# google/sbsim

Hardware: AMD Instinct MI355X
Metric: zone-updates/sec (env-steps/sec x 9 zones) at batch=64k buildings per GPU (higher is better)
Workload: dtype f64

## Files before the change

sbsim_amd/csrc/sb_device.h:

```cpp
#ifndef SBSIM_AMD_SB_DEVICE_H_
#define SBSIM_AMD_SB_DEVICE_H_

#include <hip/hip_runtime.h>

#include <stdint.h>

#include "sbsim_amd.h"

namespace sb {

constexpr double kCAir = 1006.0;
constexpr double kCWater = 4180.0;
constexpr double kRhoWater = 1000.0;
constexpr double kGravity = 9.8;
constexpr int kNScalOut = 16;
constexpr int kNScal = 20;
constexpr int kChunk = 8;
constexpr int kPad = 8;
constexpr double kAgeNone = -1e300;
__host__ __device__ inline bool age_is_none(double age) { return age < -1e200; }
constexpr int kModeMask = 0xff, kValveBit = 0x100;

struct Dev {
  int B, H, W, Z, N, Np, ncls, pitch, NL;
// ... 36 lines not shown
  int stream_ms;
  int n_ring;
  double n_ring_f64;
  int lw[4], l0[2], rowbase[2], nch[2];
  int lag;
  int nslots;
  float pred_haste;
  float pred_slack;
  int two_skip;
  float skip_kappa;
  int pred_first;
  int lds_reg_bytes;
  int wg_per_cu;
  int r_seam, r_A, r_zscr, r_xchg, r_zoff, r_zmode;
  int r_cmap;
  const unsigned long long *cmapS;
  const unsigned long long *amapS;
  const unsigned long long *zmapS;
  const int *cell_state;
  double *ring;
  double *temp;
  double *zmean;
  double *zair;
  double *damper;
  double *qz;
  int *mode;
  double *scal;
  struct Bld *bld;
  double *gtabg;
  double *zsum;
  double *gsum;
  int *nsw;
  int *next_b;
  int sweep_wgs;
  int *redo_ctr;
  int *redo_list;
  double *redo_scratch;
  int redo_mode;
  int roll_exact;
  int dbg_redo_mod;
  int O, col_ahu, col_blr, col_aux;
  const int *col_zone;
  const double *obs_mean, *obs_sigma;
  int n_src, n_hist, hist_normalize;
  const int *src_dest, *hist_col, *hist_off;
  const double *hist_bins;
  const int *act_kind, *act_zone;
  const double *act_lo, *act_hi;
  const int *zone_act;
  int n_damper_actions;
  long long *dbg;
  int dbg_timeline;
  sb_params p;
};

struct StepArgs {
  const float *actions;
  float *obs, *reward, *info;
  sb_step_in in;
};

int launch_sweep_lds(const Dev &d, int workgroups, int waves_per_wg, size_t lds_bytes, hipStream_t stream);
int prepare_sweep_lds(size_t lds_bytes);
int launch_sweep_reg(const Dev &d, int cus, hipStream_t stream);
int prepare_sweep_reg(const Dev &d);
bool sweep_reg_supported(int NR, int P);
int sweep_reg_table_stride(int NR, int P);
int sweep_reg_lds_slots(int NR, int P);
int sweep_reg_waves_per_simd(int NR, int P);
int launch_sweep_roll(const Dev &d, hipStream_t stream);
int launch_sweep_two(const Dev &d, hipStream_t stream);
int prepare_sweep_two(const Dev &d);
bool sweep_two_supported(int NR);
int sweep_two_levels();
int sweep_two_lds_slots(int NR, int level);
int sweep_two_a_stride(int NR, int level);
int sweep_two_seam_doubles(int NR);
int sweep_two_set_table();
int launch_sweep_band(const Dev &d, hipStream_t stream);
int prepare_sweep_band(const Dev &d);
bool sweep_band_supported(int NR);
int sweep_band_lds_slots(int NR);
int sweep_band_max_waves();
int sweep_band_seam_doubles(int NR, int W);
int sweep_band_sync_doubles(int W);
int sweep_band_decision_lag(int NR, int W);
int sweep_band_set_table();
int launch_sweep_stream(const Dev &d, double *abuf, int waves, hipStream_t stream);
int prepare_sweep_stream(const Dev &d, int waves);
int sweep_stream_set_table();
int sweep_stream_zone_columns();
int launch_sweep_stream_ms(const Dev &d, double *abuf, double *ebuf, int waves, hipStream_t stream);
int prepare_sweep_stream_ms(const Dev &d, int waves);
int sweep_stream_ms_sweeps();
int sweep_stream_ms_seam_doubles(int NS, int W);
int sweep_stream_ms_xchg_doubles(int W);
int prepare_sweep_roll(const Dev &d);
bool sweep_roll_supported(int NR);
int sweep_roll_lds_slots(int NR);
int sweep_roll_a_stride(int NR);
int sweep_roll_seam_doubles(int NR, int T);
int sweep_roll_waves();
int sweep_roll_tail_mul_doubles(int NR, int T);

template <int CTRL, int ROW_MASK>
__device__ __forceinline__ double dpp_or_zero(double x) {
// ... 442 lines not shown
```

sbsim_amd/csrc/sbsim_hip.hip:

```cpp
#include <hip/hip_runtime.h>

#include <algorithm>
#include <cmath>
#include <cstdio>
#include <cstdlib>
#include <cstring>
#include <memory>
#include <string>
#include <vector>

#include "sb_host.h"

#ifndef SB_EXPERIMENTAL
namespace sb {
int launch_sweep_stream_ms(const Dev &, double *, double *, int, hipStream_t) { return (int)hipErrorNotSupported; }
int prepare_sweep_stream_ms(const Dev &, int) { return (int)hipErrorNotSupported; }
int sweep_stream_ms_sweeps() { return 1; }
int sweep_stream_ms_seam_doubles(int, int) { return 0; }
int sweep_stream_ms_xchg_doubles(int) { return 0; }
}
#endif

using namespace sb;

namespace {

bool env_flag(const char *name) {
  const char *e = getenv(name);
  return e && e[0] == '1';
}
int env_int(const char *name, int unset) {
  const char *e = getenv(name);
  return e ? atoi(e) : unset;
}
double env_double(const char *name, double unset) {
  const char *e = getenv(name);
  return e ? atof(e) : unset;
}

struct Knobs {
  bool force_stream = env_flag("SBSIM_FORCE_STREAM_PATH");
  bool force_lds = env_flag("SBSIM_FORCE_LDS_PATH");
  bool band_path = env_flag("SBSIM_BAND_PATH");
  bool no_two_row = env_flag("SBSIM_NO_TWO_ROW_PATH");
  bool no_band = env_flag("SBSIM_NO_BAND_PATH");
  bool no_two_64 = env_flag("SBSIM_NO_TWO_64");
  bool no_roll_64 = env_flag("SBSIM_NO_ROLL_64");
  bool no_roll_small = env_flag("SBSIM_NO_ROLL_SMALL");
  bool two_general = env_flag("SBSIM_TWO_GENERAL");
  int two_max_level = std::max(0, env_int("SBSIM_TWO_MAX_LEVEL", 1 << 30));
  bool two_no_skip = env_flag("SBSIM_TWO_NO_SKIP");
  int lds_pad = env_int("SBSIM_DEBUG_LDS_PAD", 0);
  float pred_haste = (float)env_double("SBSIM_DEBUG_PRED_HASTE", 1.0);
  float pred_slack = (float)env_double("SBSIM_DEBUG_PRED_SLACK", 1.0);
  int pred_first = getenv("SBSIM_DEBUG_PRED_FIRST") ? std::max(1, env_int("SBSIM_DEBUG_PRED_FIRST", 1)) : 0;
  float skip_kappa = (float)std::min(100.0, std::max(0.0, env_double("SBSIM_DEBUG_SKIP_KAPPA", 0.9)));
  bool roll_exact = env_int("SBSIM_ROLL_EXACT", 0) != 0;
  int force_redo = std::max(0, env_int("SBSIM_DEBUG_FORCE_REDO", 0));
  bool force_generic = env_flag("SBSIM_FORCE_GENERIC_SWEEP");
  bool phase_timing = getenv("SBSIM_PHASE_TIMING") != nullptr;
  bool debug_timeline = getenv("SBSIM_DEBUG_TIMELINE") != nullptr;
  bool stream_ms = kExperimental && env_flag("SBSIM_STREAM_MS");
  bool stream_roll = kExperimental && env_flag("SBSIM_STREAM_ROLL");
};

constexpr int kGuardHost = 16;

struct RegPlan {
  bool ok = false;
  std::string why;
  sb_sweep_kernel kernel = SB_KERNEL_LDS;
  int NR = 0, RS = 0, Ws = 0, r0 = 0, c0 = 0, n_ring = 0, T = 0, state_doubles = 0, ts = 32;
  std::vector<uint8_t> tcls, tcset;
  std::vector<double> csetab;
  std::vector<double> tmul;
  int lw[4] = {0, 0, 0, 0}, l0[2] = {0, 0}, rowbase[2] = {0, 0}, nch[2] = {0, 0};
  int lag = 0, nslots = 0, steps = 0;
  int r_seam = 0, r_A = 0, r_xchg = 0, lds_bytes = 0, wg_per_cu = 0, AS = 0;
  int r_cmap = 0, wave_doubles = 0, waves_per_wg = 1;
  int ZRS = 0;
  int stream_variant = kStreamPlain;
  std::vector<unsigned long long> cmapS, amapS, zmapS;
  std::vector<int> cell_state;
  int two_sym = 0, two_level = 0, tail_set_base = 0, tail_pad_set = 0;
  std::vector<int> zs_off;
};

constexpr int kRegSeamPad = 8, kLdsCap = 160 * 1024;
constexpr int kLdsGranule = 1280;
constexpr int kRegSlots[] = {32, 66, 96};

int seam_lag(int lw0) { return (lw0 + 8) / 8 + 1; }

struct Trim {
  int x0, x1, y0, y1, Hs, Ws;
  std::vector<int> zone_of;
  std::string why;
};

Trim trim_box(const sb_plan_desc *plan) {
  const int H = plan->H, W = plan->W, ncls = plan->n_classes;
  auto coef = [&](int c, int j) { return plan->class_coef[c * 8 + j]; };
  auto cls_at = [&](int x, int y) { return (int)plan->cell_class[x * W + y]; };
  Trim t{H, -1, W, -1, 0, 0, std::vector<int>((size_t)H * W, -1), ""};
// ... 793 lines not shown
      return fail(SB_ERR_INVALID, "sb_create: unknown action kind");
    if (kind == SB_ACT_VAV_SUPPLY_AIR_DAMPER_COMMAND) {
      const int z = params->act_zone[i];
      if (z < 0 || z >= plan->Z) return fail(SB_ERR_INVALID, "sb_create: VAV action for a zone the floor plan does not have");
      if (acts.zone_act[z] >= 0) return fail(SB_ERR_INVALID, "sb_create: two action columns drive the same VAV damper");
      acts.zone_act[z] = i;
      ++acts.n_damper_actions;
    } else if (seen[kind]++) {
      return fail(SB_ERR_INVALID, "sb_create: two action columns drive the same setpoint");
    }
  }
  if (obs->n_obs < 1) return fail(SB_ERR_INVALID, "sb_create: empty observation layout");
  if (!obs->mean || !obs->sigma || (plan->Z > 0 && !obs->col_zone))
    return fail(SB_ERR_INVALID, "sb_create: null observation-layout table");
  {
    const int n_fields = obs->n_src ? obs->n_src : obs->n_obs, n_ahu = params->ahu_has_weather ? 9 : 8;
    bool ok = obs->col_ahu >= 0 && obs->col_ahu + n_ahu <= n_fields && obs->col_boiler >= 0 &&
              obs->col_boiler + 3 <= n_fields && obs->col_aux >= 0 && obs->col_aux + SB_NUM_AUX <= obs->n_obs;
    for (int z = 0; z < plan->Z; ++z) ok = ok && obs->col_zone[z] >= 0 && obs->col_zone[z] + 3 <= n_fields;
    if (!ok) return fail(SB_ERR_INVALID, "sb_create: observation columns outside the observation row");
  }
  for (int z = 0; z < plan->Z; ++z)
    if (plan->zone_off[z + 1] == plan->zone_off[z]) return fail(SB_ERR_INVALID, "sb_create: a zone without cells");
  if (obs->n_src) {
    const int n_dev_fields = 3 * plan->Z + (params->ahu_has_weather ? 9 : 8) + 3;
    if (obs->n_src != n_dev_fields || !obs->src_dest || obs->n_hist < 0 ||
        (obs->n_hist > 0 && (!obs->hist_col || !obs->hist_off || !obs->hist_bins)))
      return fail(SB_ERR_INVALID, "sb_create: inconsistent histogram-reducer layout");
    for (int i = 0; i < obs->n_src; ++i)
      if (obs->src_dest[i] >= obs->n_obs || obs->src_dest[i] < -obs->n_hist)
        return fail(SB_ERR_INVALID, "sb_create: histogram-reducer destination out of range");
    for (int j = 0; j < obs->n_hist; ++j) {
      const int n = obs->hist_off[j + 1] - obs->hist_off[j];
      if (n < 1 || obs->hist_col[j] < 0 || obs->hist_col[j] + n > obs->n_obs)
        return fail(SB_ERR_INVALID, "sb_create: histogram columns out of range");
    }
  }
  return SB_OK;
}

int setup_reg(sb_handle *h, const sb_plan_desc *plan, const RegPlan &r, const Knobs &k) {
  Dev &d = h->d;
  for (int g = 0; g < d.N; ++g) h->h_state_index[g] = r.cell_state[g];
  d.pitch = d.W; d.NL = d.N; d.ts = r.ts;
  d.NR = r.NR; d.RS = r.RS; d.Ws = r.Ws; d.n_ring = r.n_ring; d.n_ring_f64 = (double)r.n_ring;
  d.T = r.T; d.state_doubles = r.state_doubles; d.AS = r.AS; d.ZRS = r.ZRS ? r.ZRS : (r.RS | 1);
  for (int w = 0; w < 2; ++w) { d.l0[w] = r.l0[w]; d.rowbase[w] = r.rowbase[w]; d.nch[w] = r.nch[w]; }
  for (int w = 0; w < 4; ++w) d.lw[w] = r.lw[w];
  d.lag = r.lag; d.nslots = r.nslots; d.nsteps = r.steps;
  d.lds_reg_bytes = r.lds_bytes; d.wg_per_cu = r.wg_per_cu;
  d.r_seam = r.r_seam; d.r_A = r.r_A; d.r_xchg = r.r_xchg;
  if (h->kernel == SB_KERNEL_ROLL) { d.r_cmap = r.r_cmap; d.lds_wave_doubles = r.wave_doubles; }
  d.pred_haste = k.pred_haste; d.pred_slack = k.pred_slack;
  if (h->kernel == SB_KERNEL_TWO_ROWS && !k.two_no_skip) {
    bool mono = true;
    for (int c = 0; c < plan->n_classes; ++c) {
      double sum = 0.0;
      for (int j = 0; j < 4; ++j) { mono = mono && plan->class_coef[c * 8 + j] >= 0.0; sum += plan->class_coef[c * 8 + j]; }
      mono = mono && sum <= 1.0;
    }
    d.two_skip = mono ? 1 : 0;
  }
  d.skip_kappa = k.skip_kappa;
  d.pred_first = h->kernel == SB_KERNEL_BAND ? 2 : 3;
  if (k.pred_first) d.pred_first = k.pred_first;
  SB_CHECK(upload(h->zone_cells_l, plan->zone_cells, (size_t)plan->zone_off[plan->Z]));
  SB_CHECK(upload(h->cmapS, r.cmapS.data(), r.cmapS.size()));
  SB_CHECK(upload(h->amapS, r.amapS.data(), r.amapS.size()));
  SB_CHECK(upload(h->zmapS, r.zmapS.data(), r.zmapS.size()));
  SB_CHECK(upload(h->cell_state, r.cell_state.data(), r.cell_state.size()));
  SB_CHECK(alloc_zero(h->ring, (size_t)d.B * std::max(r.n_ring, 1)));
  SB_CHECK(upload(h->tcls, r.tcls.data(), r.tcls.size()));
  SB_CHECK(upload(h->tcset, r.tcset.data(), r.tcset.size()));
  SB_CHECK(upload(h->csetab, r.csetab.data(), r.csetab.size()));
  SB_CHECK(upload(h->tmul, r.tmul.data(), r.tmul.size()));
  d.tmulS = h->tmul.p; d.tmul_doubles = (int)r.tmul.size();
  d.tcset = h->tcset.p; d.csetab = h->csetab.p; d.ncset = (int)r.csetab.size() / 4;
  d.csetab_doubles = (int)r.csetab.size();
  d.two_sym = r.two_sym; d.two_level = r.two_level; d.tail_set_base = r.tail_set_base;
  d.tail_pad_set = h->kernel == SB_KERNEL_TWO_ROWS ? r.tail_pad_set : (d.ncset - 1) * 32;
  if (!r.zs_off.empty()) {
    SB_CHECK(upload(h->zs_off, r.zs_off.data(), r.zs_off.size()));
    d.zs_off = h->zs_off.p;
  }
  SB_CHECK(alloc_zero(h->temp, (size_t)d.B * d.state_doubles));
  if (h->kernel == SB_KERNEL_STREAM) {
    SB_CHECK(alloc_zero(h->abuf, (size_t)h->info.workgroups * d.state_doubles));
    if (h->stream_variant != kStreamPlain) SB_CHECK(alloc_zero(h->ebuf, (size_t)h->info.workgroups * d.state_doubles));
  }
  if (h->kernel == SB_KERNEL_TWO_ROWS) {
    SB_CHECK(alloc_zero(h->abuf, (size_t)h->info.workgroups * (size_t)std::max(1, d.NR - sweep_two_lds_slots(d.NR, d.two_level)) * 128));
    d.two_abuf = h->abuf.p;
  }
  if (h->kernel == SB_KERNEL_ROLL) {
    SB_CHECK(alloc_zero(h->redo_ctr, 2));
    SB_CHECK(alloc_zero(h->redo_list, (size_t)d.B));
    SB_CHECK(alloc_zero(h->redo_scratch, (size_t)h->info.workgroups * h->info.waves_per_workgroup * d.state_doubles));
    d.redo_ctr = h->redo_ctr.p; d.redo_list = h->redo_list.p; d.redo_scratch = h->redo_scratch.p;
    d.roll_exact = k.roll_exact; d.dbg_redo_mod = k.force_redo;
  }
  d.tcls = h->tcls.p;
  d.cmapS = h->cmapS.p; d.amapS = h->amapS.p; d.zmapS = h->zmapS.p; d.cell_state = h->cell_state.p;
  d.ring = h->ring.p;
  return SB_OK;
}

int setup_lds(sb_handle *h, const sb_plan_desc *plan, const LdsPlan &q, const Knobs &k) {
  Dev &d = h->d;
  for (int g = 0; g < d.N; ++g) h->h_state_index[g] = kPad + g;
  d.pitch = q.pitch; d.NL = q.NL; d.S = q.S; d.S_magic = q.S_magic; d.nsteps = q.nsteps;
  d.nbands = q.nbands; d.fast = q.fast; d.ts = q.ts;
  if (k.force_generic) d.fast = 0;
  d.off_agtab = q.off_agtab; d.off_zscr = q.off_zscr; d.off_zmode = q.off_zmode;
  d.lds_wave_doubles = q.lds_wave_doubles;
// ... 200 lines not shown
```

sbsim_amd/csrc/step_roll.hip:

```cpp
#include "sweep_common.h"

namespace sb {
namespace {

using namespace sweep;

#ifndef SB_ONE_WAIT
#define SB_ONE_WAIT 1
#endif
constexpr int kWin = 63;
constexpr int kTS = 32;
constexpr int kSeamPad = 8;

constexpr int lds_slots(int NR) { return NR >= 72 ? 72 : ((NR / 2) % 2 ? NR : NR + 2); }
constexpr int a_stride(int NR) { return NR >= 72 ? 70 : ((NR / 2) % 2 ? NR : NR + 2); }
constexpr int kWaves = 4;
constexpr int tail_row(int NR) { return NR + 4; }

struct PairBuf {
  d2 ud0, lr0, ud1, lr1;
  d2 A;
  d2 sm;
};

// ... 30 lines not shown
  unsigned off;
  if constexpr (j % 4 == 0) asm("v_lshlrev_b32_sdwa %0, 5, %1 dst_sel:DWORD dst_unused:UNUSED_PAD src0_sel:DWORD src1_sel:BYTE_0" : "=v"(off) : "v"(h));
  else if constexpr (j % 4 == 1) asm("v_lshlrev_b32_sdwa %0, 5, %1 dst_sel:DWORD dst_unused:UNUSED_PAD src0_sel:DWORD src1_sel:BYTE_1" : "=v"(off) : "v"(h));
  else if constexpr (j % 4 == 2) asm("v_lshlrev_b32_sdwa %0, 5, %1 dst_sel:DWORD dst_unused:UNUSED_PAD src0_sel:DWORD src1_sel:BYTE_2" : "=v"(off) : "v"(h));
  else asm("v_lshlrev_b32_sdwa %0, 5, %1 dst_sel:DWORD dst_unused:UNUSED_PAD src0_sel:DWORD src1_sel:BYTE_3" : "=v"(off) : "v"(h));
  return (lds_d2)off;
}

template <int NR, int S, bool SEAM, int NAR>
__device__ __forceinline__ void load_first(PairBuf &p, Ctx<NR> &x, const double (&Areg)[NAR]) {
#ifdef SB_EXP_NOCOEF
  p.ud0 = p.lr0 = x.kc;
  const lds_d2 ct = nullptr;
#else
  const lds_d2 ct = step_set<NR, S>(x);
  p.ud0 = ct[0];
#endif
#if defined(SB_EXP_ONECOEF)
  p.lr0 = p.ud0;
#elif !defined(SB_EXP_NOCOEF)
  p.lr0 = ct[1];
#endif
  constexpr int q = (S + 1) % NR, NL = lds_slots(NR), AS = a_stride(NR);
  static_assert(q % 2 == 0 && AS % 2 == 0, "pairs start at odd steps");
  if constexpr (q < AS) p.A = *(const d2 *)(x.Arow + q);
  else if constexpr (q < NL) p.A = *(const d2 *)(x.Aext + (q - AS));
  else p.A = d2{Areg[q - NL], Areg[q + 1 - NL]};
  if constexpr (SEAM && S >= kWin) p.sm = *(const d2 *)(x.seam + S);
  else p.sm = d2{0.0, 0.0};
}
template <int NR, int S>
__device__ __forceinline__ void load_second(PairBuf &p, Ctx<NR> &x) {
#ifdef SB_EXP_NOCOEF
  p.ud1 = p.lr1 = x.kc;
#else
  const lds_d2 ct = step_set<NR, S>(x);
  p.ud1 = ct[0];
#ifdef SB_EXP_ONECOEF
  p.lr1 = p.ud1;
#else
  p.lr1 = ct[1];
#endif
#endif
}

__device__ __forceinline__ void track(Acc &acc, double d) {
#ifdef SB_EXP_NOTRACK
  return;
#endif
  asm("v_max_f32 %0, %0, %1" : "+v"(acc.fin) : "v"(acc.tr));
  asm("v_max_f32_dpp %0, %0, |%1| wave_shr:1 row_mask:0xf bank_mask:0xf bound_ctrl:1" : "+v"(acc.tr) : "v"(__double2hiint(d)));
}

template <int NR, int S, bool EXACT>
__device__ __forceinline__ void step(double (&e)[NR], double (&bk)[kWin], d2 ud, d2 lr, double A,
                                     double sm, Acc &acc) {
  constexpr int r = S % NR, rm = (S + NR - 1) % NR, rp = (S + 1) % NR;
  const double Dn = wave_shift1<0x130, true>(e[rp], sm);
  double t;
  asm("v_fma_f64 %0, %1, %2, %3" : "=&v"(t) : "v"(ud.y), "v"(Dn), "v"(A));
  t = fma(lr.y, e[rp], t);
  const double U = wave_shift1<0x13c, false>(e[rm], 0.0);
  t = fma(lr.x, e[rm], t);
  const double nv = fma(ud.x, U, t);
#ifndef SB_EXP_NOSR
  if constexpr (S > kWin) {
    double &sr = (S - kWin - 1) % 2 == 0 ? acc.sre : acc.sro;
    sr = wave_shift1<0x138, true>(sr, U);
  }
#endif
  if constexpr (S < kWin) {
    const double sel = lanes_upto<S>() ? nv : e[r];
    if constexpr (EXACT) acc.cur = fmax(acc.cur, fabs(sel - e[r]));
    else track(acc, sel - e[r]);
    e[r] = sel;
  } else if constexpr (S < NR) {
    if constexpr (EXACT) acc.cur = fmax(acc.cur, fabs(nv - e[r]));
    else track(acc, nv - e[r]);
    e[r] = nv;
  } else if constexpr (!EXACT) {
    constexpr int J = S - NR;
    track(acc, nv - e[r]);
#ifndef SB_EXP_NOCOPY
    bk[J] = e[r];
#endif
    e[r] = nv;
  } else {
    constexpr int J = S - NR;
    const double d = nv - e[r];
    bk[J] = e[r];
    e[r] = nv;
    const double sd = __hiloint2double((__double2hiint(d) & 0x7fffffff) | acc.sg, __double2loint(d));
    acc.cur = fmax(acc.cur, sd);
    acc.neg = fmin(acc.neg, sd);
    if constexpr (J + 1 < kWin)
      acc.sg = __builtin_amdgcn_update_dpp(acc.sg, acc.sg, 0x138, 0xf, 0xf, false);
    asm volatile("" : "+v"(acc.cur), "+v"(acc.neg));
  }
}

constexpr int kA0 = 8;
template <int NR, int NAR>
struct APass {
  const unsigned long long (&cw)[(NR + 7) / 8];
  unsigned tbase;
  double *Aw, *Ax;
  double (&Areg)[NAR];
  template <int J>
  __device__ __forceinline__ d2 fetch() const {
    static_assert(kTS * 8 == 256, "a class byte (class * 8) is the byte offset into ap[] and into g[]");
    const unsigned h = (J & 7) < 4 ? (unsigned)cw[J >> 3] : (unsigned)(cw[J >> 3] >> 32);
    unsigned ad;
    if constexpr ((J & 3) == 0) asm("v_add_u32_sdwa %0, %1, %2 dst_sel:DWORD dst_unused:UNUSED_PAD src0_sel:DWORD src1_sel:BYTE_0" : "=v"(ad) : "s"(tbase), "v"(h));
    else if constexpr ((J & 3) == 1) asm("v_add_u32_sdwa %0, %1, %2 dst_sel:DWORD dst_unused:UNUSED_PAD src0_sel:DWORD src1_sel:BYTE_1" : "=v"(ad) : "s"(tbase), "v"(h));
    else if constexpr ((J & 3) == 2) asm("v_add_u32_sdwa %0, %1, %2 dst_sel:DWORD dst_unused:UNUSED_PAD src0_sel:DWORD src1_sel:BYTE_2" : "=v"(ad) : "s"(tbase), "v"(h));
    else asm("v_add_u32_sdwa %0, %1, %2 dst_sel:DWORD dst_unused:UNUSED_PAD src0_sel:DWORD src1_sel:BYTE_3" : "=v"(ad) : "s"(tbase), "v"(h));
    const __attribute__((address_space(3))) double *tp = (const __attribute__((address_space(3))) double *)ad;
    return d2{tp[0], tp[kTS]};
  }
  template <int J>
  __device__ __forceinline__ void put(const d2 &pg, const double &ej) const {
    constexpr int q = (J + 1) % NR, NL = lds_slots(NR), AS = a_stride(NR);
    double av;
    asm("v_fma_f64 %0, %1, %2, %3" : "=v"(av) : "v"(pg.x), "v"(ej), "v"(pg.y));
    if constexpr (q < AS) Aw[q] = av;
    else if constexpr (q < NL) Ax[q - AS] = av;
    else Areg[q - NL] = av;
  }
};

#ifndef SB_DEPTH
#define SB_DEPTH 1
#endif
constexpr int kDepth = SB_DEPTH;
constexpr int kBufs = kDepth + 1;
constexpr int pair_buf(int S) { return ((S - 1) / 2) % kBufs; }

template <int NR, int S, int S1, bool WRAP, bool EXACT, bool APASS, int NAR>
__device__ __forceinline__ void roll_pairs(double (&e)[NR], double (&bk)[kWin], double (&Areg)[NAR],
                                           PairBuf (&pb)[kBufs], Ctx<NR> &x, Acc &acc, const APass<NR, NAR> &ap) {
  if constexpr (S < S1) {
    constexpr bool wrapped = WRAP && S + 2 * kDepth >= S1;
    constexpr int N = wrapped ? S + 2 * kDepth - NR : S + 2 * kDepth;
    PairBuf &cur = pb[pair_buf(S)], &nxt = pb[pair_buf(N)];
#if SB_ONE_WAIT
    asm volatile("" ::"v"(cur.ud0.x), "v"(cur.A.x), "v"(cur.sm.x), "v"(cur.ud1.x), "v"(cur.lr1.x));
    __builtin_amdgcn_sched_barrier(0);
#endif
    load_first<NR, N, !wrapped>(nxt, x, Areg);
    constexpr int j0 = kA0 + 3 * ((S - 1) / 2);
    static_assert(!APASS || (S % 2 == 1 && j0 >= S + 2 * kDepth + 2), "a slot's A is written before the pair that reads it ahead");
    d2 pa0 = d2{0.0, 0.0}, pa1 = d2{0.0, 0.0}, pa2 = d2{0.0, 0.0};
    if constexpr (APASS && j0 < NR) pa0 = ap.template fetch<j0 < NR ? j0 : 0>();
    if constexpr (APASS && j0 + 1 < NR) pa1 = ap.template fetch<j0 + 1 < NR ? j0 + 1 : 0>();
    if constexpr (APASS && j0 + 2 < NR) pa2 = ap.template fetch<j0 + 2 < NR ? j0 + 2 : 0>();
    __builtin_amdgcn_sched_barrier(0);
    step<NR, S, EXACT>(e, bk, cur.ud0, cur.lr0, cur.A.x, cur.sm.x, acc);
    __builtin_amdgcn_sched_barrier(0);
    load_second<NR, N + 1>(nxt, x);
    __builtin_amdgcn_sched_barrier(0);
    step<NR, S + 1, EXACT>(e, bk, cur.ud1, cur.lr1, cur.A.y, cur.sm.y, acc);
    __builtin_amdgcn_sched_barrier(0);
    if constexpr (APASS && j0 < NR) ap.template put<j0 < NR ? j0 : 0>(pa0, e[j0 < NR ? j0 : 0]);
    if constexpr (APASS && j0 + 1 < NR) ap.template put<j0 + 1 < NR ? j0 + 1 : 0>(pa1, e[j0 + 1 < NR ? j0 + 1 : 0]);
    if constexpr (APASS && j0 + 2 < NR) ap.template put<j0 + 2 < NR ? j0 + 2 : 0>(pa2, e[j0 + 2 < NR ? j0 + 2 : 0]);
    if constexpr (APASS) __builtin_amdgcn_sched_barrier(0);
    roll_pairs<NR, S + 2, S1, WRAP, EXACT, APASS>(e, bk, Areg, pb, x, acc, ap);
  }
}

template <int NR, int J>
__device__ __forceinline__ void hand_over(double (&e)[NR], const double (&bk)[kWin], const unsigned long long (&zw)[NR / 8],
                                          double *tp, const double *np_, double *zrow) {
  static_assert(NR % 8 == 0, "whole zone words");
  if constexpr (J < NR) {
    if constexpr (J < kWin) e[J] = lanes_upto<J>() ? bk[J] : e[J];
    if constexpr (J + 1 < kWin) e[J + 1] = lanes_upto<J + 1>() ? bk[J + 1] : e[J + 1];
    const unsigned w = (J & 7) < 4 ? (unsigned)zw[J / 8] : (unsigned)(zw[J / 8] >> 32);
    const unsigned off0 = (w >> (8 * (J & 3))) & 0xffu, off1 = (w >> (8 * ((J + 1) & 3))) & 0xffu;
#ifndef SB_EXP_NOMEM
    __builtin_nontemporal_store(d2{e[J], e[J + 1]}, (d2 *)(tp + J * 64));
#endif
    __hip_atomic_fetch_add((double *)((char *)zrow + off0), e[J], __ATOMIC_RELAXED, __HIP_MEMORY_SCOPE_WORKGROUP);
    __hip_atomic_fetch_add((double *)((char *)zrow + off1), e[J + 1], __ATOMIC_RELAXED, __HIP_MEMORY_SCOPE_WORKGROUP);
#ifndef SB_EXP_NOMEM
    const d2 nv = __builtin_nontemporal_load((const d2 *)(np_ + J * 64));
    e[J] = nv.x;
    e[J + 1] = nv.y;
#endif
    if constexpr ((J & 7) == 6) __builtin_amdgcn_sched_barrier(0);
    hand_over<NR, J + 2>(e, bk, zw, tp, np_, zrow);
  }
}

extern __shared__ __attribute__((aligned(16))) double lds[];

template <int NR, bool EXACT>
__global__ void __launch_bounds__(64 * kWaves) __attribute__((amdgpu_waves_per_eu(1, 1))) k_sweep_roll(Dev a) {
  const int nB = a.redo_mode ? __builtin_amdgcn_readfirstlane(a.redo_ctr[0]) : a.B;
  if (nB == 0) return;
  const int lane = threadIdx.x & 63;
  const int wave = __builtin_amdgcn_readfirstlane((int)threadIdx.x >> 6);
  const int gw = (int)blockIdx.x * kWaves + wave;
  constexpr int kASlots = (NR + 7) / 8, kZSlots = NR / 8, kCW = NR / 8;
  static_assert((NR / 2) % kBufs == 0, "pair buffers rotate through a whole period: pair_buf() must not alias across the wrap");
  constexpr int kNL = lds_slots(NR), kAS = a_stride(NR), kNAR = NR - kNL > 0 ? NR - kNL : 2;

  double *tabc = lds;
  unsigned long long *ctab8 = (unsigned long long *)(lds + a.r_cmap);
  double *tmul = lds + a.r_cmap + kCW * 64;
  double *wl = tmul + a.tmul_doubles + (size_t)wave * a.lds_wave_doubles;
  double *tapg = wl;
  double *tE0 = wl + a.r_seam + 2;
  double *A = wl + a.r_A;
  for (int i = threadIdx.x; i < a.lds_reg_bytes / 8; i += blockDim.x) lds[i] = 0.0;
  __syncthreads();
  for (int i = threadIdx.x; i < 4 * kTS; i += blockDim.x) tabc[i] = i < 4 * a.ncset ? a.csetab[i] : 0.0;
  for (int i = threadIdx.x; i < kCW * 64; i += blockDim.x) ctab8[i] = a.cmapS[i];
  for (int i = threadIdx.x; i < a.tmul_doubles; i += blockDim.x) tmul[i] = a.tmulS[i];
  if (lane < kTS) tapg[lane] = lane <= a.ncls ? a.ctab[lane * 8 + 4] : 0.0;
// ... 19 lines not shown
#pragma unroll
  for (int t = 0; t < kTailMax; ++t) {
    tset[t] = (a.ncset - 1) * 32 * 0x10001;
    tcls8[t] = (8 * a.ncls) | ((8 * a.ncls) << 8);
    if (t < a.T && tactive) {
      const int c0 = tc0, c1 = tc0 + 1;
      tset[t] = ((int)a.tcset[t * NR + c0] << 2) | ((int)a.tcset[t * NR + c1] << 18);
      tcls8[t] = (int)a.tcls[t * NR + c0] | ((int)a.tcls[t * NR + c1] << 8);
    }
  }
  const unsigned long long *amap = a.amapS + lane;
  const unsigned long long *zmap = a.zmapS + lane;

#ifdef SB_PHASE_STAMPS
#define SB_STAMP(i) do { if (a.dbg && gw == 0 && iter == 10 && lane == 0) a.dbg[i] = (long long)__builtin_readcyclecounter(); } while (0)
#else
#define SB_STAMP(i) do { } while (0)
#endif

  double e[NR];
  double nx_g = 0.0, nx_tail[kTailMax][2] = {{0.0, 0.0}, {0.0, 0.0}}, nx_tnow = 0.0, nx_lo = 0.0, nx_hi = 0.0;
#define SB_LOAD_AUX(bb)                                                                         \
  do {                                                                                          \
    nx_tnow = a.bld[(bb)].t_now;                                                                \
    nx_lo = a.scal[(size_t)(bb) * kNScal + 16];                                                 \
    nx_hi = a.scal[(size_t)(bb) * kNScal + 17];                                                 \
    nx_g = a.gtabg[(size_t)(bb) * kTS + (opaque(lane) & (kTS - 1))];  \
    const double *tt_ = a.temp + (size_t)(bb) * a.state_doubles + NR * 64;                      \
    _Pragma("unroll") for (int t = 0; t < kTailMax; ++t)                                        \
      _Pragma("unroll") for (int k = 0; k < 2; ++k)                                             \
        if (t < a.T) nx_tail[t][k] = tt_[t * NR + tc0 + k];                                     \
  } while (0)
  auto building = [&](int s) { return a.redo_mode ? __builtin_amdgcn_readfirstlane(a.redo_list[s]) : s; };
  const int b_first = gw < nB ? building(gw) : 0;
  if (gw < nB) {
    const double *tp_ = a.temp + (size_t)b_first * a.state_doubles;
#pragma unroll
    for (int j = 0; j < NR; j += 2) {
      const d2 v = __builtin_nontemporal_load((const d2 *)(tp_ + j * 64 + 2 * R));
      e[j] = v.x;
      e[j + 1] = v.y;
    }
    SB_LOAD_AUX(b_first);
  }
  unsigned long long amapw[kASlots];
#define SB_LOAD_AMAP(g0, g1)                                                                    \
  do {                                                                                          \
    const int o_ = opaque(0);                                                                   \
    _Pragma("unroll") for (int g = (g0); g < (g1); ++g) amapw[g] = amap[o_ + g * 64];           \
  } while (0)
  constexpr int kAHalf = kASlots / 2;
  SB_LOAD_AMAP(0, kASlots);
  int iter = 0;
  for (int s = gw, sn = 0, b = b_first, bn = 0; s < nB; s = sn, b = bn, ++iter) {
    int nb = 0;
    if (lane == 0) nb = atomicAdd(a.next_b, 1);
    SB_STAMP(0);
    x.wn = x.cw[0];
    __builtin_amdgcn_sched_barrier(0);
    const double t_now = nx_tnow;
    const double ring_d = a.n_ring > 0 ? fmax(fabs(t_now - nx_lo), fabs(t_now - nx_hi)) : 0.0;
    if (lane < kTS) tapg[kTS + opaque(lane)] = nx_g;
    double tv[kTailMax][2];
#pragma unroll
    for (int t = 0; t < kTailMax; ++t)
#pragma unroll
      for (int k = 0; k < 2; ++k) tv[t][k] = tactive ? nx_tail[t][k] : 0.0;
    *(d2 *)(tE0 + opaque(tcw)) = d2{tv[0][0], tv[0][1]};
    __builtin_amdgcn_wave_barrier();
    __builtin_amdgcn_sched_barrier(0);
    SB_STAMP(1);
    double At[kTailMax][2] = {{0.0, 0.0}, {0.0, 0.0}};
    if constexpr (!EXACT) {
      const double *pg[kTailMax][2];
#pragma unroll
      for (int t = 0; t < kTailMax; ++t)
#pragma unroll
        for (int k = 0; k < 2; ++k) pg[t][k] = (const double *)((const char *)tapg + ((opaque(tcls8[t]) >> (8 * k)) & 0xff));
      double tap[kTailMax][2], tg[kTailMax][2];
#pragma unroll
      for (int t = 0; t < kTailMax; ++t)
#pragma unroll
        for (int k = 0; k < 2; ++k) { tap[t][k] = pg[t][k][0]; tg[t][k] = pg[t][k][kTS]; }
#pragma unroll
      for (int t = 0; t < kTailMax; ++t)
#pragma unroll
        for (int k = 0; k < 2; ++k) At[t][k] = fma(tap[t][k], tv[t][k], tg[t][k]);
    } else {
#pragma unroll
      for (int t = 0; t < kTailMax; ++t)
#pragma unroll
        for (int k = 0; k < 2; ++k)
          if (t < a.T && tactive) {
            const int c8 = (opaque(tcls8[t]) >> (8 * k)) & 0xff;
            const double *pg = (const double *)((const char *)tapg + c8);
            At[t][k] = fma(pg[0], tv[t][k], pg[kTS]);
          }
    }

    double Areg[kNAR];
    Areg[0] = 0.0;
    const APass<NR, kNAR> ap{amapw, (unsigned)(size_t)(__attribute__((address_space(3))) double *)tapg, A + (size_t)R * kAS,
                             A + 64 * kAS + (size_t)R * (kNL - kAS), Areg};
    {
      static_assert(kA0 == 8 && kA0 + 3 * ((kWin - 1) / 2) >= NR, "the ramp-up's pairs reach the last slot");
      const d2 g0 = ap.template fetch<0>(), g1 = ap.template fetch<1>(), g2 = ap.template fetch<2>(), g3 = ap.template fetch<3>(),
               g4 = ap.template fetch<4>(), g5 = ap.template fetch<5>(), g6 = ap.template fetch<6>(), g7 = ap.template fetch<7>();
      __builtin_amdgcn_sched_barrier(0);
      ap.template put<0>(g0, e[0]); ap.template put<1>(g1, e[1]); ap.template put<2>(g2, e[2]); ap.template put<3>(g3, e[3]);
      ap.template put<4>(g4, e[4]); ap.template put<5>(g5, e[5]); ap.template put<6>(g6, e[6]); ap.template put<7>(g7, e[7]);
    }
    __builtin_amdgcn_wave_barrier();
    __builtin_amdgcn_sched_barrier(0);
    SB_STAMP(2);

    int n_sweeps = 0, converged = 0, redo = 0;
    double bk[kWin];
    {
      PairBuf pb[kBufs];
      Acc acc;
      acc.cur = 0.0; acc.neg = 0.0; acc.sg = lane == 0 ? (int)0x80000000 : 0;
      acc.tr = acc.fin = 0;
      acc.sre = acc.sro = 0.0;
      {
        const lds_d2 ct = step_set<NR, 0>(x);
        const d2 ud = ct[0], lr = ct[1];
        load_first<NR, 1, true>(pb[pair_buf(1)], x, Areg);
        load_second<NR, 2>(pb[pair_buf(1)], x);
        if constexpr (kDepth > 1) {
          load_first<NR, 3, true>(pb[pair_buf(3)], x, Areg);
          load_second<NR, 4>(pb[pair_buf(3)], x);
        }
        static_assert(kDepth <= 2, "initial fill of the pair buffers");
        step<NR, 0, EXACT>(e, bk, ud, lr, x.Arow[1], 0.0, acc);
      }
      __builtin_amdgcn_sched_barrier(0);
      roll_pairs<NR, 1, kWin, false, EXACT, true>(e, bk, Areg, pb, x, acc, ap);
#ifndef SB_STAMP_NEXT
      SB_STAMP(15);
#endif
#pragma nounroll
      for (;;) {
        __builtin_amdgcn_sched_barrier(0);
#ifdef SB_PHASE_STAMPS
#ifndef SB_STAMP_SWEEP
#define SB_STAMP_SWEEP 1
#endif
#define SB_STAMP2(i) do { if (a.dbg && gw == 0 && iter == 10 && sweep_idx == SB_STAMP_SWEEP && lane == 0) a.dbg[i] = (long long)__builtin_readcyclecounter(); } while (0)
        const int sweep_idx = n_sweeps;
#ifdef SB_STAMP_NEXT
        if (a.dbg && gw == 0 && iter == 10 && sweep_idx == SB_STAMP_SWEEP + 1 && lane == 0) a.dbg[15] = (long long)__builtin_readcyclecounter();
#endif
#else
#define SB_STAMP2(i) do { } while (0)
#endif
        SB_STAMP2(10);
        roll_pairs<NR, kWin, NR + kWin, true, EXACT, false>(e, bk, Areg, pb, x, acc, ap);
        SB_STAMP2(11);
        double U0, U1;
        {
          constexpr int last = (NR + kWin - 1) % NR;
          const double ul = wave_shift1<0x13c, false>(e[last], 0.0);
          double &sr = (NR - 1) % 2 == 0 ? acc.sre : acc.sro;
          sr = wave_shift1<0x138, true>(sr, ul);
          const int rev = (63 - lane) * 4;
          U0 = __hiloint2double(__builtin_amdgcn_ds_bpermute(rev, __double2hiint(acc.sre)),
                                __builtin_amdgcn_ds_bpermute(rev, __double2loint(acc.sre)));
          U1 = __hiloint2double(__builtin_amdgcn_ds_bpermute(rev, __double2hiint(acc.sro)),
                                __builtin_amdgcn_ds_bpermute(rev, __double2loint(acc.sro)));
        }
        SB_STAMP2(12);
        const double dt_ = tail_pass_static<NR>(a.T, tmul + opaque(tc0), tE0 + opaque(tcw), U0, U1, tv, tset, At);

        SB_STAMP2(13);
        if constexpr (EXACT) {
          double md = wave_max(fmax(acc.cur, dt_));
          if (n_sweeps == 0) md = fmax(md, ring_d);
          ++n_sweeps;
          converged = md <= p.conv_threshold;
        } else {
          asm("v_max_f32 %0, %0, %1" : "+v"(acc.fin) : "v"(acc.tr));
          int m_hi = max(__builtin_amdgcn_readlane(acc.fin, 63), wave_max_i32(__double2hiint(dt_)));
          if (n_sweeps == 0) m_hi = max(m_hi, __double2hiint(ring_d));
          const int thr_hi = __double2hiint(p.conv_threshold);
          ++n_sweeps;
          acc.fin = 0;
          acc.tr = lanes_upto<62>() ? acc.tr : 0;
          const bool undecided = m_hi == thr_hi || (a.dbg_redo_mod > 0 && b % a.dbg_redo_mod == 0);
          if (m_hi <= thr_hi && undecided) { redo = 1; break; }
          converged = m_hi < thr_hi;
        }
        SB_STAMP2(14);
#ifdef SB_EXP_DESYNC
        if (n_sweeps >= 1 + (int)(((unsigned)b * 2654435761u >> 13) % 9u)) break;
#else
        if (converged || n_sweeps >= p.iter_limit) break;
#endif
        pb[pair_buf(kWin)].sm = *(const d2 *)(x.seam + kWin);
        if constexpr (kDepth > 1) pb[pair_buf(kWin + 2)].sm = *(const d2 *)(x.seam + kWin + 2);
        acc.cur = -acc.neg;
        acc.neg = 0.0;
        acc.sg = lane == 0 ? (int)0x80000000 : 0;
      }
    }
    __builtin_amdgcn_sched_barrier(0);
    SB_STAMP(3);
    sn = a.sweep_wgs + __builtin_amdgcn_readfirstlane(nb);
    bn = sn < nB ? building(sn) : 0;
    if (sn < nB) SB_LOAD_AUX(bn);
    SB_LOAD_AMAP(0, kAHalf);
    __builtin_amdgcn_sched_barrier(0);
    SB_STAMP(4);

    double *zs = A;
    const int ZRS = a.ZRS;
    {
      unsigned long long zw[kZSlots];
      const unsigned long long *zm = zmap + opaque(0);
#pragma unroll
      for (int g = 0; g < kZSlots; ++g) zw[g] = zm[g * 64];
      __builtin_amdgcn_sched_barrier(0);
      double *tp = redo ? a.redo_scratch + (size_t)gw * a.state_doubles : a.temp + (size_t)b * a.state_doubles;
      double *Ttail = tp + NR * 64;
      double *zrow = zs + (size_t)opaque(R) * ZRS;
      for (int z = 0; z <= a.Z; ++z) zrow[z] = 0.0;
      __builtin_amdgcn_wave_barrier();
#pragma unroll
      for (int t = 0; t < kTailMax; ++t)
        if (t < a.T && tactive) {
          *(d2 *)(Ttail + t * NR + tc0) = d2{tv[t][0], tv[t][1]};
          zrow[a.Z] += tv[t][0] + tv[t][1];
        }
      const double *np_ = a.temp + (size_t)(sn < nB ? bn : b) * a.state_doubles;
      static_assert(RS == 64, "hand_over: slot stride");
      hand_over<NR, 0>(e, bk, zw, tp + 2 * R, np_ + 2 * R, zrow);
    }
    __builtin_amdgcn_sched_barrier(0);
    SB_STAMP(5);
    SB_LOAD_AMAP(kAHalf, kASlots);
    __builtin_amdgcn_sched_barrier(0);
    SB_STAMP(6);
    __builtin_amdgcn_wave_barrier();
    SB_STAMP(7);

    {
      double gacc = 0.0;
      for (int zb = 0; zb <= a.Z; zb += 16) {
        const int zz = zb + (lane >> 2), g = lane & 3;
        const double *zr = zs + (size_t)g * ZRS + (zz <= a.Z ? zz : a.Z);
        double part[RS / 4];
#pragma unroll
        for (int k = 0; k < RS / 4; ++k) part[k] = zr[(size_t)4 * k * ZRS];
        double v = 0.0;
#pragma unroll
        for (int k = 0; k < RS / 4; ++k) v += part[k];
        if (zz > a.Z) v = 0.0;
        v += dpp_or_zero<0xB1, 0xf>(v);
        v += dpp_or_zero<0x4E, 0xf>(v);
        if (g == 0 && zz < a.Z && !redo) a.zsum[(size_t)b * a.Z + zz] = v;
        if (g == 0 && zz <= a.Z) gacc += v;
      }
      const double gsum = wave_sum(gacc);
      if (lane == 0 && !redo) {
        a.gsum[b] = gsum + a.n_ring_f64 * t_now;
        a.nsw[b] = n_sweeps | (converged << 16);
      }
      if (lane == 0 && redo) a.redo_list[atomicAdd(a.redo_ctr, 1)] = b;
      SB_STAMP(8);
#ifdef SB_PHASE_STAMPS
      if (a.dbg && gw == 0 && iter == 10 && lane == 0) a.dbg[9] = n_sweeps;
#endif
    }
  }
#undef SB_STAMP
#undef SB_LOAD_AUX
#undef SB_LOAD_AMAP
}

}

bool sweep_roll_supported(int NR) { return NR == 64 || NR == 72 || NR == 80 || NR == 88 || NR == 96; }
int sweep_roll_lds_slots(int NR) { return lds_slots(NR); }
int sweep_roll_a_stride(int NR) { return a_stride(NR); }
int sweep_roll_seam_doubles(int NR, int T) { (void)T; return tail_row(NR); }
int sweep_roll_waves() { return kWaves; }
int sweep_roll_tail_mul_doubles(int NR, int T) { return tail_mul_doubles(NR, T); }

int sweep_roll_redo_workgroups() { return 8; }

namespace {

template <int NR>
int prepare(const Dev &d) {
  const int e = (int)hipFuncSetAttribute((const void *)k_sweep_roll<NR, false>, hipFuncAttributeMaxDynamicSharedMemorySize,
                                         d.lds_reg_bytes);
  if (e != (int)hipSuccess) return e;
  return (int)hipFuncSetAttribute((const void *)k_sweep_roll<NR, true>, hipFuncAttributeMaxDynamicSharedMemorySize,
                                  d.lds_reg_bytes);
}

template <int NR>
int launch(const Dev &d, hipStream_t stream) {
  const dim3 grid((d.sweep_wgs + kWaves - 1) / kWaves), block(64 * kWaves);
  if (d.roll_exact) {
    hipLaunchKernelGGL((k_sweep_roll<NR, true>), grid, block, (size_t)d.lds_reg_bytes, stream, d);
    return (int)hipGetLastError();
  }
  hipLaunchKernelGGL((k_sweep_roll<NR, false>), grid, block, (size_t)d.lds_reg_bytes, stream, d);
  Dev r = d;
  r.redo_mode = 1;
  r.next_b = d.redo_ctr + 1;
  r.sweep_wgs = sweep_roll_redo_workgroups() * kWaves;
  hipLaunchKernelGGL((k_sweep_roll<NR, true>), dim3(sweep_roll_redo_workgroups()), block, (size_t)d.lds_reg_bytes, stream, r);
  return (int)hipGetLastError();
}

// ... 22 lines not shown
```

Measured before the change: 285.8 million.

## Skip convergence measurement on predicted non-converging sweeps in roll kernel

Extends the measurement-skip scheme from the two-row kernel to the roll kernel. The code extrapolates the residual decay from the last two measured sweeps, predicts how many sweeps remain, and runs those sweeps without residual tracking or backup copies. If a skipped run overshoots convergence, the building is rerun from scratch with full measurement, holding its slot instead of drawing new work. This removes per-sweep tracking and backup cost, at the price of more control flow and occasional full reruns.

```diff
diff --git a/sbsim_amd/csrc/sb_device.h b/sbsim_amd/csrc/sb_device.h
--- a/sbsim_amd/csrc/sb_device.h
+++ b/sbsim_amd/csrc/sb_device.h
@@ -112,6 +112,7 @@
   long long *dbg;
   int dbg_timeline;
   sb_params p;
+  int roll_skip;
 };
 
 struct StepArgs {
diff --git a/sbsim_amd/csrc/sbsim_hip.hip b/sbsim_amd/csrc/sbsim_hip.hip
--- a/sbsim_amd/csrc/sbsim_hip.hip
+++ b/sbsim_amd/csrc/sbsim_hip.hip
@@ -50,6 +50,7 @@
   bool two_general = env_flag("SBSIM_TWO_GENERAL");
   int two_max_level = std::max(0, env_int("SBSIM_TWO_MAX_LEVEL", 1 << 30));
   bool two_no_skip = env_flag("SBSIM_TWO_NO_SKIP");
+  bool roll_no_skip = env_flag("SBSIM_ROLL_NO_SKIP");
   int lds_pad = env_int("SBSIM_DEBUG_LDS_PAD", 0);
   float pred_haste = (float)env_double("SBSIM_DEBUG_PRED_HASTE", 1.0);
   float pred_slack = (float)env_double("SBSIM_DEBUG_PRED_SLACK", 1.0);
@@ -949,14 +950,14 @@
   d.r_seam = r.r_seam; d.r_A = r.r_A; d.r_xchg = r.r_xchg;
   if (h->kernel == SB_KERNEL_ROLL) { d.r_cmap = r.r_cmap; d.lds_wave_doubles = r.wave_doubles; }
   d.pred_haste = k.pred_haste; d.pred_slack = k.pred_slack;
-  if (h->kernel == SB_KERNEL_TWO_ROWS && !k.two_no_skip) {
+  if ((h->kernel == SB_KERNEL_TWO_ROWS && !k.two_no_skip) || (h->kernel == SB_KERNEL_ROLL && !k.roll_no_skip)) {
     bool mono = true;
     for (int c = 0; c < plan->n_classes; ++c) {
       double sum = 0.0;
       for (int j = 0; j < 4; ++j) { mono = mono && plan->class_coef[c * 8 + j] >= 0.0; sum += plan->class_coef[c * 8 + j]; }
       mono = mono && sum <= 1.0;
     }
-    d.two_skip = mono ? 1 : 0;
+    (h->kernel == SB_KERNEL_ROLL ? d.roll_skip : d.two_skip) = mono ? 1 : 0;
   }
   d.skip_kappa = k.skip_kappa;
   d.pred_first = h->kernel == SB_KERNEL_BAND ? 2 : 3;
diff --git a/sbsim_amd/csrc/step_roll.hip b/sbsim_amd/csrc/step_roll.hip
--- a/sbsim_amd/csrc/step_roll.hip
+++ b/sbsim_amd/csrc/step_roll.hip
@@ -106,9 +106,10 @@
   asm("v_max_f32_dpp %0, %0, |%1| wave_shr:1 row_mask:0xf bank_mask:0xf bound_ctrl:1" : "+v"(acc.tr) : "v"(__double2hiint(d)));
 }
 
-template <int NR, int S, bool EXACT>
+template <int NR, int S, bool EXACT, bool MEAS = true>
 __device__ __forceinline__ void step(double (&e)[NR], double (&bk)[kWin], d2 ud, d2 lr, double A,
                                      double sm, Acc &acc) {
+  static_assert(MEAS || (!EXACT && S >= kWin), "only the library kernel's rolling periods run measure-free");
   constexpr int r = S % NR, rm = (S + NR - 1) % NR, rp = (S + 1) % NR;
   const double Dn = wave_shift1<0x130, true>(e[rp], sm);
   double t;
@@ -130,14 +131,17 @@
     e[r] = sel;
   } else if constexpr (S < NR) {
     if constexpr (EXACT) acc.cur = fmax(acc.cur, fabs(nv - e[r]));
-    else track(acc, nv - e[r]);
+    else if constexpr (MEAS) track(acc, nv - e[r]);
     e[r] = nv;
   } else if constexpr (!EXACT) {
     constexpr int J = S - NR;
-    track(acc, nv - e[r]);
+    if constexpr (MEAS) {
+      track(acc, nv - e[r]);
 #ifndef SB_EXP_NOCOPY
-    bk[J] = e[r];
-#endif
+      bk[J] = e[r];
+#endif
+    }
+    (void)J;
     e[r] = nv;
   } else {
     constexpr int J = S - NR;
@@ -190,7 +194,7 @@
 constexpr int kBufs = kDepth + 1;
 constexpr int pair_buf(int S) { return ((S - 1) / 2) % kBufs; }
 
-template <int NR, int S, int S1, bool WRAP, bool EXACT, bool APASS, int NAR>
+template <int NR, int S, int S1, bool WRAP, bool EXACT, bool APASS, bool MEAS = true, int NAR>
 __device__ __forceinline__ void roll_pairs(double (&e)[NR], double (&bk)[kWin], double (&Areg)[NAR],
                                            PairBuf (&pb)[kBufs], Ctx<NR> &x, Acc &acc, const APass<NR, NAR> &ap) {
   if constexpr (S < S1) {
@@ -209,17 +213,17 @@
     if constexpr (APASS && j0 + 1 < NR) pa1 = ap.template fetch<j0 + 1 < NR ? j0 + 1 : 0>();
     if constexpr (APASS && j0 + 2 < NR) pa2 = ap.template fetch<j0 + 2 < NR ? j0 + 2 : 0>();
     __builtin_amdgcn_sched_barrier(0);
-    step<NR, S, EXACT>(e, bk, cur.ud0, cur.lr0, cur.A.x, cur.sm.x, acc);
+    step<NR, S, EXACT, MEAS>(e, bk, cur.ud0, cur.lr0, cur.A.x, cur.sm.x, acc);
     __builtin_amdgcn_sched_barrier(0);
     load_second<NR, N + 1>(nxt, x);
     __builtin_amdgcn_sched_barrier(0);
-    step<NR, S + 1, EXACT>(e, bk, cur.ud1, cur.lr1, cur.A.y, cur.sm.y, acc);
+    step<NR, S + 1, EXACT, MEAS>(e, bk, cur.ud1, cur.lr1, cur.A.y, cur.sm.y, acc);
     __builtin_amdgcn_sched_barrier(0);
     if constexpr (APASS && j0 < NR) ap.template put<j0 < NR ? j0 : 0>(pa0, e[j0 < NR ? j0 : 0]);
     if constexpr (APASS && j0 + 1 < NR) ap.template put<j0 + 1 < NR ? j0 + 1 : 0>(pa1, e[j0 + 1 < NR ? j0 + 1 : 0]);
     if constexpr (APASS && j0 + 2 < NR) ap.template put<j0 + 2 < NR ? j0 + 2 : 0>(pa2, e[j0 + 2 < NR ? j0 + 2 : 0]);
     if constexpr (APASS) __builtin_amdgcn_sched_barrier(0);
-    roll_pairs<NR, S + 2, S1, WRAP, EXACT, APASS>(e, bk, Areg, pb, x, acc, ap);
+    roll_pairs<NR, S + 2, S1, WRAP, EXACT, APASS, MEAS>(e, bk, Areg, pb, x, acc, ap);
   }
 }
 
@@ -345,9 +349,11 @@
   constexpr int kAHalf = kASlots / 2;
   SB_LOAD_AMAP(0, kASlots);
   int iter = 0;
+  int held = -1;
   for (int s = gw, sn = 0, b = b_first, bn = 0; s < nB; s = sn, b = bn, ++iter) {
     int nb = 0;
-    if (lane == 0) nb = atomicAdd(a.next_b, 1);
+    if (lane == 0 && (EXACT || held < 0)) nb = atomicAdd(a.next_b, 1);
+    const bool all_meas = held >= 0;
     SB_STAMP(0);
     x.wn = x.cw[0];
     __builtin_amdgcn_sched_barrier(0);
@@ -407,7 +413,7 @@
     __builtin_amdgcn_sched_barrier(0);
     SB_STAMP(2);
 
-    int n_sweeps = 0, converged = 0, redo = 0;
+    int n_sweeps = 0, converged = 0, redo = 0, rerun = 0;
     double bk[kWin];
     {
       PairBuf pb[kBufs];
@@ -432,21 +438,62 @@
 #ifndef SB_STAMP_NEXT
       SB_STAMP(15);
 #endif
+#ifdef SB_PHASE_STAMPS
+#ifndef SB_STAMP_SWEEP
+#define SB_STAMP_SWEEP 1
+#endif
+#define SB_STAMP2(i) do { if (a.dbg && gw == 0 && iter == 10 && sweep_idx == SB_STAMP_SWEEP && lane == 0) a.dbg[i] = (long long)__builtin_readcyclecounter(); } while (0)
+#else
+#define SB_STAMP2(i) do { } while (0)
+#endif
+      int ha = 0, hb = 0, sa = 0, sb = 0, nh = 0, next_meas = 0;
 #pragma nounroll
       for (;;) {
         __builtin_amdgcn_sched_barrier(0);
-#ifdef SB_PHASE_STAMPS
-#ifndef SB_STAMP_SWEEP
-#define SB_STAMP_SWEEP 1
-#endif
-#define SB_STAMP2(i) do { if (a.dbg && gw == 0 && iter == 10 && sweep_idx == SB_STAMP_SWEEP && lane == 0) a.dbg[i] = (long long)__builtin_readcyclecounter(); } while (0)
         const int sweep_idx = n_sweeps;
 #ifdef SB_STAMP_NEXT
         if (a.dbg && gw == 0 && iter == 10 && sweep_idx == SB_STAMP_SWEEP + 1 && lane == 0) a.dbg[15] = (long long)__builtin_readcyclecounter();
 #endif
-#else
-#define SB_STAMP2(i) do { } while (0)
-#endif
+        bool whole = true;
+        if constexpr (!EXACT) {
+          int nskip = 0;
+          if (a.roll_skip && !all_meas && nh >= 2) nskip = min(next_meas, p.iter_limit - 1) - (n_sweeps + 1);
+          nskip = __builtin_amdgcn_readfirstlane(nskip);
+#pragma nounroll
+          for (int i = 0; i < nskip; ++i) {
+            __builtin_amdgcn_sched_barrier(0);
+            const int sweep_idx = n_sweeps;
+#ifdef SB_PHASE_STAMPS
+            if (a.dbg && gw == 0 && iter == 10 && sweep_idx == SB_STAMP_SWEEP && lane == 0) a.dbg[14] = 0;
+#endif
+            SB_STAMP2(10);
+            roll_pairs<NR, kWin, NR + kWin, true, EXACT, false, false>(e, bk, Areg, pb, x, acc, ap);
+            SB_STAMP2(11);
+            {
+              double U0, U1;
+              {
+                constexpr int last = (NR + kWin - 1) % NR;
+                const double ul = wave_shift1<0x13c, false>(e[last], 0.0);
+                double &sr = (NR - 1) % 2 == 0 ? acc.sre : acc.sro;
+                sr = wave_shift1<0x138, true>(sr, ul);
+                const int rev = (63 - lane) * 4;
+                U0 = __hiloint2double(__builtin_amdgcn_ds_bpermute(rev, __double2hiint(acc.sre)),
+                                      __builtin_amdgcn_ds_bpermute(rev, __double2loint(acc.sre)));
+                U1 = __hiloint2double(__builtin_amdgcn_ds_bpermute(rev, __double2hiint(acc.sro)),
+                                      __builtin_amdgcn_ds_bpermute(rev, __double2loint(acc.sro)));
+              }
+              SB_STAMP2(12);
+              (void)tail_pass_static<NR>(a.T, tmul + opaque(tc0), tE0 + opaque(tcw), U0, U1, tv, tset, At);
+            }
+            SB_STAMP2(13);
+            ++n_sweeps;
+            pb[pair_buf(kWin)].sm = *(const d2 *)(x.seam + kWin);
+            if constexpr (kDepth > 1) pb[pair_buf(kWin + 2)].sm = *(const d2 *)(x.seam + kWin + 2);
+            __builtin_amdgcn_sched_barrier(0);
+          }
+          whole = nskip <= 0;
+          if (!whole) acc.tr = 0;
+        }
         SB_STAMP2(10);
         roll_pairs<NR, kWin, NR + kWin, true, EXACT, false>(e, bk, Areg, pb, x, acc, ap);
         SB_STAMP2(11);
@@ -479,9 +526,23 @@
           ++n_sweeps;
           acc.fin = 0;
           acc.tr = lanes_upto<62>() ? acc.tr : 0;
-          const bool undecided = m_hi == thr_hi || (a.dbg_redo_mod > 0 && b % a.dbg_redo_mod == 0);
-          if (m_hi <= thr_hi && undecided) { redo = 1; break; }
-          converged = m_hi < thr_hi;
+          if (whole) {
+            const bool undecided = m_hi == thr_hi || (a.dbg_redo_mod > 0 && b % a.dbg_redo_mod == 0);
+            if (m_hi <= thr_hi && undecided) { redo = 1; break; }
+            converged = m_hi < thr_hi;
+            if (!converged && a.roll_skip) {
+              ha = hb; sa = sb;
+              hb = m_hi; sb = n_sweeps;
+              nh = nh < 2 ? nh + 1 : 2;
+              const float da = (float)__hiloint2double(ha, 0), db = (float)__hiloint2double(hb, 0);
+              const float togo = db < da ? fminf(__log2f((float)p.conv_threshold / db) * (float)(sb - sa) / __log2f(db / da), 1000.0f) : 1.0f;
+              const int ahead = (int)(a.skip_kappa * togo) - 1;
+              next_meas = __builtin_amdgcn_readfirstlane(n_sweeps + (ahead > 1 ? ahead : 1));
+            }
+          } else {
+            if (m_hi <= __double2hiint(p.conv_threshold + 1e-9)) { rerun = 1; break; }
+            converged = 0;
+          }
         }
         SB_STAMP2(14);
 #ifdef SB_EXP_DESYNC
@@ -498,7 +559,18 @@
     }
     __builtin_amdgcn_sched_barrier(0);
     SB_STAMP(3);
-    sn = a.sweep_wgs + __builtin_amdgcn_readfirstlane(nb);
+    if constexpr (EXACT) {
+      sn = a.sweep_wgs + __builtin_amdgcn_readfirstlane(nb);
+    } else {
+      const int drawn = held >= 0 ? held : a.sweep_wgs + __builtin_amdgcn_readfirstlane(nb);
+      held = -1;
+      if (rerun) {
+        held = drawn;
+        sn = s;
+      } else {
+        sn = drawn;
+      }
+    }
     bn = sn < nB ? building(sn) : 0;
     if (sn < nB) SB_LOAD_AUX(bn);
     SB_LOAD_AMAP(0, kAHalf);
@@ -513,7 +585,7 @@
 #pragma unroll
       for (int g = 0; g < kZSlots; ++g) zw[g] = zm[g * 64];
       __builtin_amdgcn_sched_barrier(0);
-      double *tp = redo ? a.redo_scratch + (size_t)gw * a.state_doubles : a.temp + (size_t)b * a.state_doubles;
+      double *tp = redo || rerun ? a.redo_scratch + (size_t)gw * a.state_doubles : a.temp + (size_t)b * a.state_doubles;
       double *Ttail = tp + NR * 64;
       double *zrow = zs + (size_t)opaque(R) * ZRS;
       for (int z = 0; z <= a.Z; ++z) zrow[z] = 0.0;
@@ -550,11 +622,11 @@
         if (zz > a.Z) v = 0.0;
         v += dpp_or_zero<0xB1, 0xf>(v);
         v += dpp_or_zero<0x4E, 0xf>(v);
-        if (g == 0 && zz < a.Z && !redo) a.zsum[(size_t)b * a.Z + zz] = v;
+        if (g == 0 && zz < a.Z && !redo && !rerun) a.zsum[(size_t)b * a.Z + zz] = v;
         if (g == 0 && zz <= a.Z) gacc += v;
       }
       const double gsum = wave_sum(gacc);
-      if (lane == 0 && !redo) {
+      if (lane == 0 && !redo && !rerun) {
         a.gsum[b] = gsum + a.n_ring_f64 * t_now;
         a.nsw[b] = n_sweeps | (converged << 16);
       }
```

Result: slower. 279.3 million, median of 6 (-2.3%).
